# kabkabm/defensegan

Measured on NVIDIA H100. Metric: reconstructed images/sec at R=10,L=200, higher is better.
Workload: dtype f16

## Files before the change

### defensegan_b200/csrc/kernels_tc2.cuh

```cuda
#pragma once
#include "kernels_tc.cuh"
#include "tc_records.cuh"

namespace dgan {

constexpr int TC2_SMEM_MAX = 232448;
constexpr int TC2_TILE_BYTES = 128 * 128;
constexpr int TC2_BUF_COLS = 256;
constexpr int TC2_CONSUMERS = 256;
constexpr int TC2_THREADS = TC2_CONSUMERS + 128;
constexpr int TC2_PRODUCER_REGS = 40, TC2_CONSUMER_REGS = 232;
constexpr int TC2_STORE_ROWS = 16;

constexpr int TC2_MAX_PAIRS = 80;
struct Tc2Heads {
  uint32_t off[TC2_MAX_PAIRS + 1];
};

struct __align__(16) TcItem2 {
  uint16_t q[16];
  uint32_t n_acc;
};
static_assert(sizeof(TcItem2) == 48 && offsetof(TcItem2, n_acc) == 32, "the kernel's item loads");

__host__ __device__ constexpr int tc2_acc_stride(int n_tile) { return n_tile <= 32 ? 32 : (n_tile < 64 ? 64 : n_tile); }

__host__ __device__ constexpr bool tc2_tma_epilogue(int n_tile, int epi, int out_bytes) {
  return out_bytes == 2 && n_tile >= 64 && !tc_final_epi(epi);
}

constexpr int TC2_REC_BATCH = 16;
constexpr int TC2_STAGING_BYTES = TC2_REC_BATCH * (int)sizeof(TcRec);
constexpr int TC2_MREC_BYTES = TC2_NSLOT * (int)sizeof(TcRec);

__host__ __device__ constexpr int tc2_epi_tiles(int n_tile, int epi, int out_bytes) {
  return tc2_tma_epilogue(n_tile, epi, out_bytes) ? 2 : 0;
}
__host__ __device__ constexpr int tc2_ksub(int K) { return K % 64 == 0 ? 4 : K / 16; }
__host__ __device__ constexpr int tc2_a_bytes(int ksub) { return 128 * 32 * ksub; }
__host__ __device__ constexpr int tc2_b_bytes(int n_tile, int ksub) { return n_tile * 32 * ksub; }
__host__ __device__ constexpr bool tc2_issues_zero_ops(int maxb, int ksub) { return maxb > 4 || (maxb > 1 && ksub < 4); }
__host__ __device__ constexpr int tc2_zero_bytes(int n_tile, int maxb, int ksub) { return maxb > 1 ? tc2_b_bytes(n_tile, ksub) : 0; }
__host__ __device__ constexpr int tc2_ring_bytes(int n_tile, int maxb, int ksub, int epi, int out_bytes) {
  const int epi_b = tc2_epi_tiles(n_tile, epi, out_bytes) * TC2_TILE_BYTES;
  const int raw = ((TC2_SMEM_MAX - 1024 - 256 - TC2_MREC_BYTES - TC2_STAGING_BYTES - epi_b - tc2_zero_bytes(n_tile, maxb, ksub)) / 1024) * 1024;
  return raw > TC2_RING_MAX_KB * 1024 ? TC2_RING_MAX_KB * 1024 : raw;
}

template <int N_TILE, int MAXB_, int KSUB_ = 4, int EPI = EPI_NONE, int OUT_BYTES = 2>
struct Tc2Cfg {
  static_assert(MAXB_ >= 1 && MAXB_ <= TC2_BUF_COLS / tc2_acc_stride(N_TILE), "more accumulator slots than columns");
  static_assert(KSUB_ >= 1 && KSUB_ <= 4, "k16 MMAs per op");
  static constexpr int KSUB = KSUB_;
  static constexpr int A_BYTES = tc2_a_bytes(KSUB);
  static constexpr int B_TILE = tc2_b_bytes(N_TILE, KSUB);
  static constexpr int A_SUB = 128 * 32, B_SUB = N_TILE * 32;
  static constexpr int MAXB = MAXB_;
  static constexpr int ACC_REGS = MAXB * N_TILE / 2;
  static constexpr bool TMA_EPI = tc2_tma_epilogue(N_TILE, EPI, OUT_BYTES);
  static constexpr int EPI_TILES = tc2_epi_tiles(N_TILE, EPI, OUT_BYTES);
  static constexpr int EPI_BYTES = EPI_TILES * TC2_TILE_BYTES;
  static constexpr int ZERO_BYTES = tc2_zero_bytes(N_TILE, MAXB, KSUB);
  static constexpr int RING_BYTES = tc2_ring_bytes(N_TILE, MAXB, KSUB, EPI, OUT_BYTES);
  static constexpr int SMEM_BYTES = RING_BYTES + ZERO_BYTES + EPI_BYTES + TC2_STAGING_BYTES + 1024 + 256 + TC2_MREC_BYTES;
};

#define TC2_KINDS(X)                                                                                                   \
  X(256, 1, 4, EPI_BIAS_RELU, __half) X(256, 1, 4, EPI_BIAS, __half) X(256, 1, 4, EPI_MASK, __half)                    \
  X(256, 1, 4, EPI_NONE, __half) X(256, 1, 4, EPI_NONE, float) X(256, 1, 4, EPI_BIAS, float)                           \
  X(128, 2, 4, EPI_BIAS_RELU, __half) X(128, 2, 4, EPI_BIAS, __half) X(128, 2, 4, EPI_MASK, __half)                    \
  X(128, 2, 4, EPI_NONE, __half) X(128, 2, 4, EPI_NONE, float) X(128, 2, 4, EPI_BIAS, float)                           \
  X(128, 1, 4, EPI_NONE, float)                                                                                        \
  X(64, 4, 4, EPI_BIAS_RELU, __half) X(64, 4, 4, EPI_BIAS, __half) X(64, 4, 4, EPI_MASK, __half)                      \
  X(64, 4, 4, EPI_NONE, __half) X(64, 4, 4, EPI_NONE, float) X(64, 4, 4, EPI_BIAS, float)                              \
  X(64, 4, 1, EPI_MASK, __half) X(64, 4, 1, EPI_NONE, __half) X(64, 4, 3, EPI_NONE, __half)                            \
  X(128, 2, 1, EPI_MASK, __half) X(128, 2, 1, EPI_NONE, __half) X(128, 2, 3, EPI_NONE, __half)                         \
  X(16, 8, 4, EPI_FINAL_SIGMOID1, __half) X(16, 4, 4, EPI_FINAL_SIGMOID1, __half) X(48, 4, 4, EPI_FINAL_TANH3, __half)   \
  X(16, 8, 4, EPI_NONE, float) X(48, 4, 4, EPI_NONE, float)                                                              \
  X(16, 8, 4, EPI_FINAL_SIGMOID1_W, __half) X(16, 4, 4, EPI_FINAL_SIGMOID1_W, __half) X(48, 4, 4, EPI_FINAL_TANH3_W, __half)   \
  X(16, 8, 4, EPI_FINAL_SIGMOID1_H, __half) X(16, 4, 4, EPI_FINAL_SIGMOID1_H, __half) X(48, 4, 4, EPI_FINAL_TANH3_H, __half)   \
  X(16, 8, 4, EPI_FINAL_SIGMOID1_WH, __half) X(16, 4, 4, EPI_FINAL_SIGMOID1_WH, __half) X(48, 4, 4, EPI_FINAL_TANH3_WH, __half)

struct Tc2Kind { int n, maxb, ksub, epi, out_bytes; };
#define TC2_KIND_ROW(NT, MB, KS, EP, T) {NT, MB, KS, EP, (int)sizeof(T)},
static constexpr Tc2Kind kTc2Kinds[] = {TC2_KINDS(TC2_KIND_ROW)};
#undef TC2_KIND_ROW
constexpr bool tc2_kinds_fit_records() {
  for (const Tc2Kind& k : kTc2Kinds)
    if ((uint32_t)k.maxb > TcMmaRec::MaxB::mask || (uint32_t)k.ksub > TcMmaRec::Ksub::mask) return false;
  return true;
}
static_assert(tc2_kinds_fit_records(), "an instantiation's MAXB or KSUB does not fit the MMA record");
static inline bool tc2_has_kind(int n, int maxb, int ksub, int epi, int out_bytes) {
  for (const Tc2Kind& k : kTc2Kinds)
    if (k.n == n && k.maxb == maxb && k.ksub == ksub && k.epi == epi && k.out_bytes == out_bytes) return true;
  return false;
}

namespace ptx {
__device__ __forceinline__ void tma_store_3d(const CUtensorMap* map, uint32_t src, int c0, int c1, int c2) {
  asm volatile("cp.async.bulk.tensor.3d.global.shared::cta.tile.bulk_group [%0, {%2, %3, %4}], [%1];"
               ::"l"(map), "r"(src), "r"(c0), "r"(c1), "r"(c2) : "memory");
}
__device__ __forceinline__ void bulk_commit() { asm volatile("cp.async.bulk.commit_group;" ::: "memory"); }
__device__ __forceinline__ void bulk_wait_read1() { asm volatile("cp.async.bulk.wait_group.read 1;" ::: "memory"); }
__device__ __forceinline__ void bulk_wait_all0() { asm volatile("cp.async.bulk.wait_group 0;" ::: "memory"); }
__device__ __forceinline__ void fence_proxy_async_smem() { asm volatile("fence.proxy.async.shared::cta;" ::: "memory"); }
__device__ __forceinline__ uint32_t cluster_ctarank() {
  uint32_t r;
  asm volatile("mov.u32 %0, %%cluster_ctarank;" : "=r"(r));
  return r;
}
__device__ __forceinline__ void cluster_sync() {
  asm volatile("barrier.cluster.arrive.release.aligned;\n\tbarrier.cluster.wait.acquire.aligned;" ::: "memory");
}
__device__ __forceinline__ void tma_load_3d_mc2(uint32_t dst, const CUtensorMap* map, uint32_t bar, int c0, int c1, int c2) {
  asm volatile(
      "cp.async.bulk.tensor.3d.shared::cluster.global.mbarrier::complete_tx::bytes.multicast::cluster [%0], [%1, {%3, %4, %5}], [%2], %6;"
      ::"r"(dst), "l"(map), "r"(bar), "r"(c0), "r"(c1), "r"(c2), "h"((uint16_t)3) : "memory");
}
__device__ __forceinline__ void mbar_arrive_cluster(uint32_t local_bar, uint32_t cta) {
  asm volatile(
      "{\n\t.reg .b32 ra;\n\t"
      "mapa.shared::cluster.u32 ra, %0, %1;\n\t"
      "mbarrier.arrive.shared::cluster.b64 _, [ra];\n\t}" ::"r"(local_bar), "r"(cta) : "memory");
}
__device__ __forceinline__ void named_bar_sync(uint32_t id, uint32_t nthreads) {
  asm volatile("bar.sync %0, %1;" ::"r"(id), "r"(nthreads) : "memory");
}
__device__ __forceinline__ void st_shared_v4(uint32_t addr, uint32_t a, uint32_t b, uint32_t c, uint32_t d) {
  asm volatile("st.shared.v4.b32 [%0], {%1, %2, %3, %4};" ::"r"(addr), "r"(a), "r"(b), "r"(c), "r"(d) : "memory");
}
__device__ __forceinline__ void st_shared_u32(uint32_t addr, uint32_t v) { asm volatile("st.shared.b32 [%0], %1;" ::"r"(addr), "r"(v) : "memory"); }
__device__ __forceinline__ uint32_t ld_shared_u32(uint32_t addr) {
  uint32_t v;
  asm volatile("ld.shared.b32 %0, [%1];" : "=r"(v) : "r"(addr) : "memory");
  return v;
}
__device__ __forceinline__ uint2 ld_shared_v2(uint32_t addr) {
  uint2 v;
  asm volatile("ld.shared.v2.b32 {%0, %1}, [%2];" : "=r"(v.x), "=r"(v.y) : "r"(addr));
  return v;
}
__device__ __forceinline__ uint4 ld_shared_v4(uint32_t addr) {
  uint4 v;
  asm volatile("ld.shared.v4.b32 {%0, %1, %2, %3}, [%4];" : "=r"(v.x), "=r"(v.y), "=r"(v.z), "=r"(v.w) : "r"(addr));
  return v;
}
__device__ __forceinline__ uint4 ld_shared_v4_ordered(uint32_t addr) {
  uint4 v;
  asm volatile("ld.shared.v4.b32 {%0, %1, %2, %3}, [%4];" : "=r"(v.x), "=r"(v.y), "=r"(v.z), "=r"(v.w) : "r"(addr) : "memory");
  return v;
}
__device__ __forceinline__ void bulk_load(uint32_t dst, const void* src, uint32_t bytes, uint32_t bar) {
  asm volatile("cp.async.bulk.shared::cluster.global.mbarrier::complete_tx::bytes [%0], [%1], %2, [%3];"
               ::"r"(dst), "l"(src), "r"(bytes), "r"(bar) : "memory");
}
__device__ __forceinline__ void wgmma_wait1() { asm volatile("wgmma.wait_group.sync.aligned 1;" ::: "memory"); }
template <int R> __device__ __forceinline__ void setmaxnreg_inc() { asm volatile("setmaxnreg.inc.sync.aligned.u32 %0;" ::"n"(R)); }
template <int R> __device__ __forceinline__ void setmaxnreg_dec() { asm volatile("setmaxnreg.dec.sync.aligned.u32 %0;" ::"n"(R)); }
__device__ __forceinline__ bool elect_one() {
  uint32_t pred;
  asm volatile("{\n\t.reg .pred P1;\n\telect.sync _|P1, 0xffffffff;\n\tselp.u32 %0, 1, 0, P1;\n\t}" : "=r"(pred));
  return pred != 0;
}
}

__device__ __forceinline__ int tc2_item_at(const int* __restrict__ order, int k, int pair, int n_pairs, int n_slots) {
  return k < n_slots ? __ldg(order + (size_t)k * n_pairs + pair) : -1;
}

template <int NT, int MAXB, int KSUB, uint32_t MASK, int NREG>
__device__ __forceinline__ void tc2_mma_ops(float (&acc)[NREG], const uint32_t (&q)[6], uint64_t da0, uint64_t db0, uint32_t zoff) {
  constexpr uint32_t DA_K = KSUB == 4 ? 2u : (uint32_t)(128 * 32 >> 4), DB_K = KSUB == 4 ? 2u : (uint32_t)(NT * 32 >> 4);
#pragma unroll
  for (int a = 0; a < MAXB; ++a) {
    if (!((MASK >> a) & 1u)) continue;
    const uint32_t e = TcMmaRec::Ops::get(q[a / TcMmaRec::Ops::PER_WORD], a);
    const uint32_t bs = TcOp::Slot::get(e);
    const uint64_t da = da0 + (uint64_t)(TcOp::A::get(e) * (uint32_t)(tc2_a_bytes(KSUB) >> 4));
    const uint32_t boff = bs * (uint32_t)(tc2_b_bytes(NT, KSUB) >> 4);
    const uint64_t db = db0 + (uint64_t)(tc2_issues_zero_ops(MAXB, KSUB) && bs == (uint32_t)TC2_ZERO_SLOT ? zoff : boff);
    const uint32_t keep = TcOp::First::get(e) ^ 1u;
#pragma unroll
    for (int k = 0; k < KSUB; ++k) ptx::Wgmma<NT>::mma(acc + a * (NT / 2), da + DA_K * k, db + DB_K * k, k > 0 ? 1u : keep);
  }
  ptx::wgmma_commit();
}

template <int NT, int MAXB, int KSUB, int NREG>
__device__ __forceinline__ void tc2_mma_round(float (&acc)[NREG], const uint32_t (&q)[6], uint64_t da0, uint64_t db0, uint32_t zoff) {
  if constexpr (tc2_issues_zero_ops(MAXB, KSUB) || MAXB == 1) {
    tc2_mma_ops<NT, MAXB, KSUB, (1u << MAXB) - 1u>(acc, q, da0, db0, zoff);
  } else {
    static_assert(MAXB <= TcMmaRec::Ops::PER_WORD, "a round's op bytes share the queue's first word");
    uint32_t set = 0;
#pragma unroll
    for (int a = 0; a < MAXB; ++a)
      set |= (TcOp::Slot::get(TcMmaRec::Ops::get(q[0], a)) != (uint32_t)TC2_ZERO_SLOT ? 1u : 0u) << a;
    switch (set) {
#define TC2_ROUND_VARIANT(M) \
  case M:                    \
    if constexpr (M < (1u << MAXB)) tc2_mma_ops<NT, MAXB, KSUB, M>(acc, q, da0, db0, zoff); \
    break;
      TC2_ROUND_VARIANT(1u) TC2_ROUND_VARIANT(2u) TC2_ROUND_VARIANT(3u) TC2_ROUND_VARIANT(4u) TC2_ROUND_VARIANT(5u)
      TC2_ROUND_VARIANT(6u) TC2_ROUND_VARIANT(7u) TC2_ROUND_VARIANT(8u) TC2_ROUND_VARIANT(9u) TC2_ROUND_VARIANT(10u)
      TC2_ROUND_VARIANT(11u) TC2_ROUND_VARIANT(12u) TC2_ROUND_VARIANT(13u) TC2_ROUND_VARIANT(14u) TC2_ROUND_VARIANT(15u)
#undef TC2_ROUND_VARIANT
      default: __builtin_unreachable();
    }
  }
}

template <int MAXB>
__device__ __forceinline__ void tc2_pop_round(uint32_t (&q)[6]) {
  using Ops = TcMmaRec::Ops;
  static_assert(Ops::WORDS == 6, "the op queue holds every op word");
  if constexpr (MAXB >= Ops::PER_WORD) {
#pragma unroll
    for (int i = 0; i < 6; ++i) q[i] = (i + MAXB / Ops::PER_WORD < 6) ? q[i + MAXB / Ops::PER_WORD] : 0u;
  } else {
#pragma unroll
    for (int i = 0; i < 5; ++i) q[i] = __funnelshift_r(q[i], q[i + 1], Ops::BITS * MAXB);
    q[5] >>= Ops::BITS * MAXB;
  }
}

#ifdef DGAN_PROBE
constexpr int TC2_PROBE_WORDS = 18;
__device__ unsigned long long g_tc2_probe[48][160][TC2_PROBE_WORDS];
__device__ __forceinline__ unsigned long long probe_gtime() {
  unsigned long long t;
  asm volatile("mov.u64 %0, %%globaltimer;" : "=l"(t));
  return t;
}
__device__ __forceinline__ long long probe_clock_after(uint32_t w0) {
  long long t;
  asm volatile("{\n\t.reg .pred p;\n\tsetp.ge.s32 p, %1, 0;\n\tmov.u64 %0, 0;\n\t@p mov.u64 %0, %%clock64;\n\t}" : "=l"(t) : "r"(w0) : "memory");
  return t;
}
__device__ __forceinline__ long long probe_clock_after64(unsigned long long v) {
  long long t;
  asm volatile("{\n\t.reg .pred p;\n\tsetp.eq.u64 p, %1, 0;\n\t@p mov.u64 %0, %%clock64;\n\t@!p mov.u64 %0, %%clock64;\n\t}"
               : "=l"(t) : "l"(v) : "memory");
  return t;
}
__device__ __forceinline__ unsigned long long probe_bits(float2 v) {
  return ((unsigned long long)__float_as_uint(v.y) << 32) | __float_as_uint(v.x);
}
__host__ __device__ constexpr int tc2_probe_key(int n_tile, int epi, int out_bytes) {
  if (epi >= EPI_FINAL_SIGMOID1_H) return 40 + epi - EPI_FINAL_SIGMOID1_H;
  return (n_tile == 256 ? 0 : n_tile == 128 ? 1 : n_tile == 64 ? 2 : n_tile == 48 ? 3 : 4) * 8 + (out_bytes == 4 ? 6 : (epi < 4 ? epi : epi - 4));
}
#endif

template <int N_TILE, int MAXB, int KSUB, int EPI, typename TOUT>
__global__ void __cluster_dims__(2, 1, 1) __launch_bounds__(TC2_THREADS, 1)
tc_bsgemm2_kernel(const __grid_constant__ CUtensorMap tm_a, const __grid_constant__ CUtensorMap tm_b,
                  const __grid_constant__ CUtensorMap tm_out,
                  const TcItem2* __restrict__ items, const TcRec* __restrict__ stream_p,
                  const TcRec* __restrict__ stream_m, const __grid_constant__ Tc2Heads heads,
                  const int* __restrict__ eitems, int n_slots,
                  TOUT* __restrict__ out, int n_pad, const float* __restrict__ bias, int bias_pstride, const TcFinalArgs fa) {
  using Cfg = Tc2Cfg<N_TILE, MAXB, KSUB, EPI, (int)sizeof(TOUT)>;
  constexpr bool TMA_EPI = Cfg::TMA_EPI;
  constexpr bool HUBER = (EPI == EPI_FINAL_SIGMOID1_H || EPI == EPI_FINAL_TANH3_H || EPI == EPI_FINAL_SIGMOID1_WH ||
                          EPI == EPI_FINAL_TANH3_WH);
  constexpr bool WEIGHTED = (EPI == EPI_FINAL_SIGMOID1_W || EPI == EPI_FINAL_TANH3_W || EPI == EPI_FINAL_SIGMOID1_WH ||
                             EPI == EPI_FINAL_TANH3_WH);
  constexpr bool FINAL = tc_final_epi(EPI);
  constexpr bool SIGMOID1 = (EPI == EPI_FINAL_SIGMOID1 || EPI == EPI_FINAL_SIGMOID1_W || EPI == EPI_FINAL_SIGMOID1_H ||
                             EPI == EPI_FINAL_SIGMOID1_WH);
  constexpr bool HAS_BIAS = (EPI == EPI_BIAS_RELU || EPI == EPI_BIAS);
  constexpr int B_TILE = Cfg::B_TILE, A_BYTES = Cfg::A_BYTES;
  constexpr int PRODUCER = TC2_CONSUMERS / 32;
  extern __shared__ uint8_t smem_raw[];
#ifdef DGAN_PROBE
  const long long probe_t_start = clock64();
  const unsigned long long probe_g_start = probe_gtime();
  long long probe_wait_full = 0, probe_issue = 0, probe_wait1 = 0, probe_wait0 = 0, probe_epi = 0, probe_in = 0, probe_stage = 0;
  unsigned probe_rec = 0, probe_head = 0, probe_steps = 0;
#endif
  const uint32_t smem_base = (ptx::smem_u32(smem_raw) + 1023u) & ~1023u;
  const uint32_t zero_base = smem_base + Cfg::RING_BYTES;
  const uint32_t epi_base = zero_base + Cfg::ZERO_BYTES;
  const uint32_t stg_base = epi_base + Cfg::EPI_BYTES;
  const uint32_t bar_base = stg_base + TC2_STAGING_BYTES;
  const uint32_t bar_full = bar_base, bar_empty = bar_base + 64, mrec_base = bar_base + 256;

  const int warp = threadIdx.x >> 5, lane = threadIdx.x & 31;
  const uint32_t rank = ptx::cluster_ctarank();
  const int pair = blockIdx.x >> 1, n_pairs = gridDim.x >> 1;
  const uint32_t rbeg = heads.off[pair], rend = heads.off[pair + 1];

  uint4 mine = make_uint4(0, 0, 0, 0);
  if (warp == PRODUCER) {
    if (2 * rbeg + lane < 2 * rend) mine = __ldg(reinterpret_cast<const uint4*>(stream_p + rbeg) + lane);
    if (lane == 0) {
      ptx::prefetch_tmap(&tm_a);
      ptx::prefetch_tmap(&tm_b);
      if (TMA_EPI) ptx::prefetch_tmap(&tm_out);
      for (int s = 0; s < TC2_NSLOT; ++s) {
        ptx::mbar_init(bar_full + 8 * s, 1);
        ptx::mbar_init(bar_empty + 8 * s, 2 * TC2_CONSUMERS / 32);
      }
      ptx::fence_barrier_init();
    }
  }
  if constexpr (Cfg::ZERO_BYTES > 0 && tc2_issues_zero_ops(MAXB, KSUB)) {
    if (threadIdx.x < TC2_CONSUMERS) {
      for (uint32_t i = threadIdx.x; i < (uint32_t)Cfg::ZERO_BYTES / 16u; i += TC2_CONSUMERS) ptx::st_shared_v4(zero_base + 16u * i, 0u, 0u, 0u, 0u);
      ptx::fence_proxy_async_smem();
    }
  }
  ptx::cluster_sync();
#ifdef DGAN_PROBE
  const long long probe_t_entry = clock64();
#endif
  pdl_launch_dependents();
  pdl_wait();
#ifdef DGAN_PROBE
  const long long probe_t_go = clock64();
  unsigned probe_h0 = (unsigned)probe_t_go;
  bool probe_new_item = true;
#endif

  if (warp >= PRODUCER) {
    ptx::setmaxnreg_dec<TC2_PRODUCER_REGS>();
    if (warp == PRODUCER) {
      const TcRec* __restrict__ stream = stream_p;
      uint32_t it = 0;
      const uint32_t ring = stg_base;
      for (uint32_t base = rbeg; base < rend; base += TC2_REC_BATCH) {
        ptx::st_shared_v4(ring + lane * 16u, mine.x, mine.y, mine.z, mine.w);
        __syncwarp();
        if (2 * (base + TC2_REC_BATCH) + lane < 2 * rend) mine = __ldg(reinterpret_cast<const uint4*>(stream + base + TC2_REC_BATCH) + lane);
        const uint32_t cnt = min((uint32_t)TC2_REC_BATCH, rend - base);
        for (uint32_t i = 0; i < cnt; ++i, ++it) {
          const uint4 r0 = ptx::ld_shared_v4(ring + i * 32u);
          const uint2 r1 = ptx::ld_shared_v2(ring + i * 32u + 16u);
          const uint32_t slot = it & (TC2_NSLOT - 1);
          using P = TcProducerRec;
          const int kc = P::Kc::get(r0.x), nA = P::NA::get(r0.x), nB = P::NB::get(r0.x);
          const uint32_t dep = (r0.x >> P::Dep::shift) & P::Dep::mask;
          const int row0 = (2 * (int)P::Mp::get(r0.y) + (int)rank) * kRowTile;
          if (it >= dep) ptx::mbar_wait(bar_empty + 8 * ((it - dep) & (TC2_NSLOT - 1)), ((it - dep) >> 3) & 1);
          if (dep != TC2_NSLOT && it >= TC2_NSLOT) ptx::mbar_wait(bar_empty + 8 * slot, ((it - TC2_NSLOT) >> 3) & 1);
          const uint32_t full = bar_full + 8 * slot;
          const uint32_t sa = smem_base + (P::Off::get(r0.x) << 10);
          if (ptx::elect_one()) {
            ptx::mbar_expect_tx(full, (uint32_t)(nA * A_BYTES + nB * B_TILE) + (uint32_t)sizeof(TcRec));
            ptx::bulk_load(mrec_base + slot * (uint32_t)sizeof(TcRec), stream_m + rbeg + it, (uint32_t)sizeof(TcRec), full);
#pragma unroll
            for (int a = 0; a < TC2_MAX_A; ++a) {
              if (a >= nA) break;
              const int p = (int)P::Pix::get(a < P::Pix::PER_WORD ? r0.z : r0.w, a);
              if constexpr (KSUB == 4) {
                ptx::tma_load_3d(sa + a * A_BYTES, &tm_a, full, kc * 64, row0, p);
              } else {
#pragma unroll
                for (int k = 0; k < KSUB; ++k)
                  ptx::tma_load_3d(sa + a * A_BYTES + k * Cfg::A_SUB, &tm_a, full, (kc * KSUB + k) * 16, row0, p);
              }
            }
            const uint32_t sb = sa + nA * A_BYTES;
#pragma unroll
            for (int b = 0; b < TC2_MAX_BSLOTS; ++b) {
              if (b >= nB) break;
              const uint32_t t = P::Tile::get(b < P::Tile::PER_WORD ? r1.x : r1.y, b);
              if constexpr (KSUB == 4) {
                ptx::tma_load_3d_mc2(sb + b * B_TILE + rank * (B_TILE / 2), &tm_b, full, kc * 64, (int)rank * (N_TILE / 2), (int)t);
              } else {
#pragma unroll
                for (int k = 0; k < KSUB; ++k)
                  ptx::tma_load_3d_mc2(sb + b * B_TILE + k * Cfg::B_SUB + rank * (Cfg::B_SUB / 2), &tm_b, full, (kc * KSUB + k) * 16,
                                       (int)rank * (N_TILE / 2), (int)t);
              }
            }
          }
          __syncwarp();
        }
        __syncwarp();
      }
      for (uint32_t j = it > TC2_NSLOT ? it - TC2_NSLOT : 0; j < it; ++j) ptx::mbar_wait(bar_empty + 8 * (j & (TC2_NSLOT - 1)), (j >> 3) & 1);
    }
  } else {
    ptx::setmaxnreg_inc<TC2_CONSUMER_REGS>();
    const int wg = warp >> 2, wl = warp & 3;
    const int r_lo = wg * 64 + wl * 16 + (lane >> 2);
    float acc[Cfg::ACC_REGS];
#pragma unroll
    for (int i = 0; i < Cfg::ACC_REGS; ++i) acc[i] = 0.f;
    uint32_t item_count = 0, store_count = 0;
    uint32_t ri = rbeg, it = 0;
    auto item_desc = [&](int e, int& n, uint32_t& qm) {
      n = 0; qm = 0u;
      if (e < 0) return;
      const TcItem2* ip = items + tc2_item_window(e);
      n = (int)__ldg(&ip->n_acc);
      if (lane < 16) qm = (uint32_t)__ldg(&ip->q[lane]);
    };
    int e_cur = tc2_item_at(eitems, 0, pair, n_pairs, n_slots), e_nx = tc2_item_at(eitems, 1, pair, n_pairs, n_slots), n_acc_cur;
    uint32_t q_cur;
    item_desc(e_cur, n_acc_cur, q_cur);
    constexpr bool BIAS_CH = HAS_BIAS && TMA_EPI && N_TILE < 256, BIAS_PX = HAS_BIAS && TMA_EPI && !BIAS_CH;
    static_assert(!BIAS_CH || (Cfg::ZERO_BYTES >= N_TILE * 4 && !tc2_issues_zero_ops(MAXB, KSUB)), "the bias copy's space");
    static_assert(!BIAS_PX || MAXB == 1, "a per-pixel bias is held for one accumulator");
    if constexpr (BIAS_CH) {
      if (threadIdx.x < N_TILE / 2) {
        const float2 b2 = __ldg(reinterpret_cast<const float2*>(bias) + threadIdx.x);
        ptx::st_shared_u32(zero_base + 8u * threadIdx.x, __float_as_uint(b2.x));
        ptx::st_shared_u32(zero_base + 8u * threadIdx.x + 4u, __float_as_uint(b2.y));
      }
      ptx::named_bar_sync(4, TC2_CONSUMERS);
    }
    constexpr int CO = SIGMOID1 ? 1 : 3, FJ = FINAL ? N_TILE / 8 : 1;
    constexpr bool FINAL_PREFETCH = !(WEIGHTED && N_TILE > 32);
    constexpr int FINAL_HELD = FINAL && N_TILE <= 32 && !(WEIGHTED && MAXB > 4) ? MAXB : 1;
    const int hwc = fa.w_out * fa.w_out * CO;
    float bsv[CO];
    if constexpr (FINAL) {
#pragma unroll
      for (int co = 0; co < CO; ++co) bsv[co] = __ldg(bias + co);
    }
    while (ri < rend) {
      const int item_e = e_cur, n_acc = n_acc_cur;
      const uint32_t q_mine = q_cur;
      const int mp = tc2_item_mp(item_e);
      const int tile_row0 = (2 * mp + (int)rank) * kRowTile;
      const size_t n_lo = (size_t)(tile_row0 + r_lo);
      constexpr int G_UNITS = TMA_EPI ? N_TILE / 64 : 1;
      static_assert(EPI != EPI_MASK || MAXB * G_UNITS == 4, "one mask unit per lane of a quad");
      unsigned long long mk_pre[2] = {~0ull, ~0ull};
// ... 26 lines not shown
          xv[j] = make_float2(0.f, 0.f);
          if (fa.x != nullptr) xv[j] = __ldg(reinterpret_cast<const float2*>(fa.x + (size_t)img * hwc + off));
          wv[j] = make_float2(1.f, 1.f);
          if (WEIGHTED) wv[j] = __ldg(reinterpret_cast<const float2*>(fa.xw + (size_t)img * hwc + off));
        }
      };
      float2 xp[FINAL_HELD][2][FJ], wp[FINAL_HELD][2][FJ];
      if constexpr (FINAL && FINAL_PREFETCH) {
#pragma unroll
        for (int a = 0; a < FINAL_HELD; ++a) {
          if (a >= n_acc) break;
          final_pairs(a, 0, xp[a][0], wp[a][0]);
          final_pairs(a, 1, xp[a][1], wp[a][1]);
        }
      }
      item_desc(e_nx, n_acc_cur, q_cur);
      e_cur = e_nx;
      e_nx = tc2_item_at(eitems, (int)item_count + 2, pair, n_pairs, n_slots);
      uint32_t flags;
      do {
        const uint32_t slot = it & (TC2_NSLOT - 1), phase = (it >> 3) & 1;
#ifdef DGAN_PROBE
        const long long probe_w0 = clock64();
        if (probe_new_item) probe_head += (unsigned)probe_w0 - probe_h0;
        probe_new_item = false;
#endif
        ptx::mbar_wait(bar_full + 8 * slot, phase);
#ifdef DGAN_PROBE
        const long long probe_w1 = clock64();
        probe_wait_full += probe_w1 - probe_w0;
        if (it == 0 && threadIdx.x == 0) g_tc2_probe[tc2_probe_key(N_TILE, EPI, (int)sizeof(TOUT))][blockIdx.x][7] = probe_gtime();
#endif
        const uint4 r0 = ptx::ld_shared_v4_ordered(mrec_base + slot * (uint32_t)sizeof(TcRec));
        const uint4 r1 = ptx::ld_shared_v4_ordered(mrec_base + slot * (uint32_t)sizeof(TcRec) + 16u);
        flags = TcMmaRec::Flags::get(r0.x);
#ifdef DGAN_PROBE
        const unsigned probe_rec_step = (unsigned)probe_clock_after(r0.x) - (unsigned)probe_w1;
        probe_rec += probe_rec_step;
#endif
        const int nA = TcMmaRec::NA::get(r0.x), n_rounds = TcMmaRec::Rounds::get(r0.x);
        const uint32_t sa = smem_base + (TcMmaRec::Off::get(r0.x) << 10);
        const uint64_t da0 = KSUB == 4 ? make_smem_desc_sw128(sa + (uint32_t)wg * 64u * 128u) : make_smem_desc_sw32(sa + (uint32_t)wg * 64u * 32u);
        const uint32_t sb = sa + (uint32_t)nA * A_BYTES;
        const uint64_t db0 = KSUB == 4 ? make_smem_desc_sw128(sb) : make_smem_desc_sw32(sb);
        const uint32_t zoff = (zero_base - sb) >> 4;
        uint32_t q[6] = {r0.z, r0.w, r1.x, r1.y, r1.z, r1.w};
#ifdef DGAN_PROBE
        long long probe_step_wait = 0;
#endif
        ptx::fence_operands(acc);
        ptx::wgmma_fence();
        for (int r = 0; r < n_rounds; ++r) {
          tc2_mma_round<N_TILE, Cfg::MAXB, KSUB>(acc, q, da0, db0, zoff);
          tc2_pop_round<Cfg::MAXB>(q);
#ifdef DGAN_PROBE
          const long long probe_c0 = clock64();
#endif
          ptx::wgmma_wait1();
#ifdef DGAN_PROBE
          probe_step_wait += clock64() - probe_c0;
#endif
          if (r == 0) {
            __syncwarp();
            if (!(flags & TcMmaRec::FIRST) && lane < 2) ptx::mbar_arrive_cluster(bar_empty + 8 * ((it - 1) & (TC2_NSLOT - 1)), (uint32_t)lane);
          }
        }
        ptx::fence_operands(acc);
#ifdef DGAN_PROBE
        probe_wait1 += probe_step_wait;
        probe_issue += clock64() - probe_w1 - probe_step_wait - probe_rec_step;
#endif
        ++ri; ++it;
      } while (!(flags & TcMmaRec::LAST));
#ifdef DGAN_PROBE
      const long long probe_d0 = clock64();
#endif
      ptx::wgmma_wait0();
      ptx::fence_operands(acc);
#ifdef DGAN_PROBE
      const long long probe_e0 = clock64();
      probe_wait0 += probe_e0 - probe_d0;
#endif
      __syncwarp();
      if (lane < 2) ptx::mbar_arrive_cluster(bar_empty + 8 * ((it - 1) & (TC2_NSLOT - 1)), (uint32_t)lane);

      auto q_of = [&](int a) { return (int)__shfl_sync(0xffffffffu, q_mine, a); };
      if constexpr (FINAL) {
#pragma unroll
        for (int a = 0; a < Cfg::MAXB; ++a) {
          if (a >= n_acc) break;
          const int blk = q_of(a);
          const int by = blk / fa.nbx, bx = blk % fa.nbx;
#ifdef DGAN_PROBE
          const long long probe_a0 = clock64();
#endif
#pragma unroll
          for (int h = 0; h < 2; ++h) {
            float2 xa[FJ], wa[FJ];
            if constexpr (FINAL_PREFETCH) {
#pragma unroll
              for (int j = 0; j < FJ; ++j) { xa[j] = xp[a % FINAL_HELD][h][j]; wa[j] = wp[a % FINAL_HELD][h][j]; }
              if (FINAL_HELD == 1 && a + 1 < Cfg::MAXB && a + 1 < n_acc) final_pairs(a + 1, h, xp[0][h], wp[0][h]);
            } else {
              final_pairs(a, h, xa, wa);
            }
#ifdef DGAN_PROBE
            if (h == 0) probe_in += probe_clock_after64(probe_bits(xa[0]) ^ probe_bits(wa[0])) - probe_a0;
#endif
            const size_t n = n_lo + 8 * h;
            float lsum = 0.f;
#pragma unroll
            for (int j = 0; j < N_TILE / 8; ++j) {
              const int col = j * 8 + (lane & 3) * 2;
              const int li = col / (4 * CO), e = col % (4 * CO);
              const size_t off = (size_t)((4 * by + li) * fa.w_out + 4 * bx) * CO + e;
              const float2 xv = xa[j], wv = wa[j];
              float yv[2], dv[2];
#pragma unroll
              for (int c = 0; c < 2; ++c) {
                const float pre = acc[a * (N_TILE / 2) + j * 4 + h * 2 + c] + bsv[(e + c) % CO];
                float yy, dact;
                if (SIGMOID1) { yy = __fdividef(1.f, 1.f + __expf(-pre)); dact = yy * (1.f - yy); }
                else { const float t = __expf(-2.f * fabsf(pre)); yy = copysignf(__fdividef(1.f - t, 1.f + t), pre); dact = 1.f - yy * yy; }
                yv[c] = yy;
                float d = 0.f;
                if (HUBER) {
                  d = yy - (c ? xv.y : xv.x);
                  const float cl = fabsf(d) > fa.huber ? copysignf(fa.huber, d) : d;
                  const float ew = WEIGHTED ? (c ? wv.y : wv.x) * cl : cl;
                  lsum = fmaf(ew, 2.f * d - cl, lsum);
                  d = ew;
                } else if (WEIGHTED) {
                  d = yy - (c ? xv.y : xv.x);
                  const float ew = (c ? wv.y : wv.x) * d;
                  lsum = fmaf(ew, d, lsum);
                  d = ew;
                } else if (fa.x != nullptr) { d = yy - (c ? xv.y : xv.x); lsum = fmaf(d, d, lsum); }
                dv[c] = d * dact * fa.gscale;
              }
              if (fa.write_y) *reinterpret_cast<float2*>(fa.y + n * hwc + off) = make_float2(yv[0], yv[1]);
              if (fa.x != nullptr)
                *reinterpret_cast<uint32_t*>(reinterpret_cast<__half*>(out) + ((size_t)blk * n_pad + n) * N_TILE + col) = pack_half2(dv[0], dv[1]);
            }
            lsum += __shfl_xor_sync(0xffffffffu, lsum, 1);
            lsum += __shfl_xor_sync(0xffffffffu, lsum, 2);
            if (fa.x != nullptr && fa.write_y && (lane & 3) == 0) fa.loss_part[(size_t)blk * n_pad + n] = lsum;
          }
        }
      } else if constexpr (TMA_EPI) {
        constexpr int G = N_TILE / 64;
        const int GT = fa.out_ld >> 6;
        const int row_w = tile_row0 + wg * 64 + wl * 16;
        const uint32_t s_warp = epi_base + (uint32_t)warp * 4096u;
        const uint32_t swz = (uint32_t)(lane >> 2);
#pragma unroll
        for (int a = 0; a < Cfg::MAXB; ++a) {
          if (a >= n_acc) break;
          const int q = q_of(a);
#pragma unroll
          for (int g = 0; g < G; ++g) {
#ifdef DGAN_PROBE
            const long long probe_u0 = clock64();
#endif
            unsigned long long mk[2] = {~0ull, ~0ull}, bits[2] = {0ull, 0ull};
            if (EPI == EPI_MASK) {
#pragma unroll
              for (int h = 0; h < 2; ++h) mk[h] = __shfl_sync(0xffffffffu, mk_pre[h], (lane & ~3) | (a * G + g));
#ifdef DGAN_PROBE
              probe_in += probe_clock_after64(mk[0] ^ mk[1]) - probe_u0;
#endif
            }
            uint32_t pk[2][8];
#pragma unroll
            for (int j = 0; j < 8; ++j) {
              const int cl = j * 8 + (lane & 3) * 2;
              float2 bv = make_float2(0.f, 0.f);
              if constexpr (BIAS_CH) {
                const uint2 b2 = ptx::ld_shared_v2(zero_base + (uint32_t)(g * 64 + cl) * 4u);
                bv = make_float2(__uint_as_float(b2.x), __uint_as_float(b2.y));
              }
              if constexpr (BIAS_PX) {
                bv.x = __shfl_sync(0xffffffffu, bias_px[g].x, j * 4 + (lane & 3));
                bv.y = __shfl_sync(0xffffffffu, bias_px[g].y, j * 4 + (lane & 3));
              }
#ifdef DGAN_PROBE
              if (HAS_BIAS && j == 0) probe_in += probe_clock_after64(probe_bits(bv)) - probe_u0;
#endif
#pragma unroll
              for (int h = 0; h < 2; ++h) {
                float v0 = acc[a * (N_TILE / 2) + (g * 8 + j) * 4 + h * 2];
                float v1 = acc[a * (N_TILE / 2) + (g * 8 + j) * 4 + h * 2 + 1];
                if (HAS_BIAS) { v0 += bv.x; v1 += bv.y; }
                if (EPI == EPI_BIAS_RELU) {
                  v0 = fmaxf(v0, 0.f); v1 = fmaxf(v1, 0.f);
                  bits[h] |= ((unsigned long long)(v0 > 0.f) << cl) | ((unsigned long long)(v1 > 0.f) << (cl + 1));
                }
                if (EPI == EPI_MASK) {
                  if (!((mk[h] >> cl) & 1ull)) v0 = 0.f;
                  if (!((mk[h] >> (cl + 1)) & 1ull)) v1 = 0.f;
                }
                pk[h][j] = pack_half2(v0, v1);
              }
            }
            const uint32_t buf = s_warp + (store_count & 1u) * 2048u;
#ifdef DGAN_PROBE
            const long long probe_s0 = clock64();
#endif
            if (lane == 0) ptx::bulk_wait_read1();
            __syncwarp();
#ifdef DGAN_PROBE
            probe_stage += clock64() - probe_s0;
#endif
#pragma unroll
            for (int h = 0; h < 2; ++h)
#pragma unroll
              for (int j = 0; j < 8; ++j)
                ptx::st_shared_u32(buf + (swz + 8u * h) * 128u + (((uint32_t)j ^ swz) << 4) + (uint32_t)(lane & 3) * 4u, pk[h][j]);
            ptx::fence_proxy_async_smem();
            __syncwarp();
            if (lane == 0) {
              ptx::tma_store_3d(&tm_out, buf, fa.col0 + g * 64, row_w, q);
              ptx::bulk_commit();
            }
            ++store_count;
            if (EPI == EPI_BIAS_RELU && fa.mb_out != nullptr) {
#pragma unroll
              for (int h = 0; h < 2; ++h) {
                bits[h] |= __shfl_xor_sync(0xffffffffu, bits[h], 1);
                bits[h] |= __shfl_xor_sync(0xffffffffu, bits[h], 2);
              }
              if ((lane & 3) < 2) fa.mb_out[((size_t)q * n_pad + n_lo + 8 * (lane & 1)) * GT + g] = (lane & 1) ? bits[1] : bits[0];
            }
          }
        }
      } else {
#pragma unroll
        for (int a = 0; a < Cfg::MAXB; ++a) {
          if (a >= n_acc) break;
          const int q = q_of(a);
#pragma unroll
          for (int j = 0; j < N_TILE / 8; ++j) {
            const int col = j * 8 + (lane & 3) * 2;
            float2 bv = make_float2(0.f, 0.f);
            if (HAS_BIAS) bv = __ldg(reinterpret_cast<const float2*>(bias + (size_t)q * bias_pstride + col));
#pragma unroll
            for (int h = 0; h < 2; ++h) {
              float v0 = acc[a * (N_TILE / 2) + j * 4 + h * 2] + bv.x, v1 = acc[a * (N_TILE / 2) + j * 4 + h * 2 + 1] + bv.y;
              if (EPI == EPI_BIAS_RELU) { v0 = fmaxf(v0, 0.f); v1 = fmaxf(v1, 0.f); }
              const size_t o = ((size_t)q * n_pad + n_lo + 8 * h) * fa.out_ld + col;
              if (sizeof(TOUT) == 4) *reinterpret_cast<float2*>(reinterpret_cast<float*>(out) + o) = make_float2(v0, v1);
              else *reinterpret_cast<uint32_t*>(reinterpret_cast<__half*>(out) + o) = pack_half2(v0, v1);
            }
          }
        }
      }
      if (EPI == EPI_NONE && sizeof(TOUT) == 4 && fa.m_counter != nullptr) {
        const uint32_t flag_addr = bar_base + 200;
        const unsigned rt = 2u * (unsigned)mp + rank;
        __threadfence();
        ptx::named_bar_sync(3, TC2_CONSUMERS);
        if (threadIdx.x == 0) {
          const unsigned ticket = atomicAdd(fa.m_counter + rt, 1u);
          ptx::st_shared_u32(flag_addr, ticket == (unsigned)TC_LINEAR_SPLIT - 1u ? 1u : 0u);
        }
        ptx::named_bar_sync(3, TC2_CONSUMERS);
        if (ptx::ld_shared_u32(flag_addr) != 0u) {
          __threadfence();
          const float* __restrict__ gp = reinterpret_cast<const float*>(out);
          const size_t base = (size_t)rt * kRowTile * N_TILE;
          const int tid = threadIdx.x;
          constexpr int STRIDE = 4 * TC2_CONSUMERS, UNR = 4;
          for (int e0 = tid * 4; e0 < kRowTile * N_TILE; e0 += UNR * STRIDE) {
            float4 gs[UNR], vv[UNR], zz[UNR];
#pragma unroll
            for (int u = 0; u < UNR; ++u) {
              const size_t i = base + (size_t)(e0 + u * STRIDE);
              gs[u] = __ldcg(reinterpret_cast<const float4*>(gp + i));
              vv[u] = *reinterpret_cast<const float4*>(fa.mv + i);
              zz[u] = *reinterpret_cast<const float4*>(fa.mz + i);
            }
            float4 t[TC_LINEAR_SPLIT - 1][UNR];
#pragma unroll
            for (int pp = 1; pp < TC_LINEAR_SPLIT; ++pp)
#pragma unroll
              for (int u = 0; u < UNR; ++u)
                t[pp - 1][u] = __ldcg(reinterpret_cast<const float4*>(gp + base + (size_t)(e0 + u * STRIDE) + (size_t)pp * fa.m_count));
#pragma unroll
            for (int pp = 1; pp < TC_LINEAR_SPLIT; ++pp)
#pragma unroll
              for (int u = 0; u < UNR; ++u) { gs[u].x += t[pp - 1][u].x; gs[u].y += t[pp - 1][u].y; gs[u].z += t[pp - 1][u].z; gs[u].w += t[pp - 1][u].w; }
#pragma unroll
            for (int u = 0; u < UNR; ++u) {
              const size_t i = base + (size_t)(e0 + u * STRIDE);
              float4 v4 = vv[u], z4 = zz[u];
              v4.x = fmaf(fa.m_mu, v4.x, fa.m_gmul * gs[u].x); v4.y = fmaf(fa.m_mu, v4.y, fa.m_gmul * gs[u].y);
              v4.z = fmaf(fa.m_mu, v4.z, fa.m_gmul * gs[u].z); v4.w = fmaf(fa.m_mu, v4.w, fa.m_gmul * gs[u].w);
              z4.x -= fa.m_lr * v4.x; z4.y -= fa.m_lr * v4.y; z4.z -= fa.m_lr * v4.z; z4.w -= fa.m_lr * v4.w;
              *reinterpret_cast<float4*>(fa.mv + i) = v4;
              *reinterpret_cast<float4*>(fa.mz + i) = z4;
              if (fa.mz_h != nullptr)
                *reinterpret_cast<uint2*>(fa.mz_h + i) = make_uint2(pack_half2(z4.x, z4.y), pack_half2(z4.z, z4.w));
            }
          }
          if (tid == 0) fa.m_counter[rt] = 0u;
        }
      }
#ifdef DGAN_PROBE
      const long long probe_e1 = clock64();
      probe_epi += probe_e1 - probe_e0;
      probe_h0 = (unsigned)probe_e1;
      probe_new_item = true;
      probe_steps = it;
#endif
      ++item_count;
    }
    if (TMA_EPI && lane == 0) ptx::bulk_wait_all0();
  }

#ifdef DGAN_PROBE
  {
    constexpr int key = tc2_probe_key(N_TILE, EPI, (int)sizeof(TOUT));
    if (threadIdx.x == 0) {
      atomicAdd(&g_tc2_probe[key][blockIdx.x][3], (unsigned long long)probe_wait_full);
      atomicAdd(&g_tc2_probe[key][blockIdx.x][8], (unsigned long long)probe_issue);
      atomicAdd(&g_tc2_probe[key][blockIdx.x][9], (unsigned long long)probe_wait1);
      atomicAdd(&g_tc2_probe[key][blockIdx.x][10], (unsigned long long)probe_wait0);
      atomicAdd(&g_tc2_probe[key][blockIdx.x][11], (unsigned long long)probe_epi);
      atomicAdd(&g_tc2_probe[key][blockIdx.x][16], (unsigned long long)probe_in);
      atomicAdd(&g_tc2_probe[key][blockIdx.x][17], (unsigned long long)probe_stage);
    }
    __syncthreads();
    if (threadIdx.x == 0) {
      atomicAdd(&g_tc2_probe[key][blockIdx.x][12], (unsigned long long)probe_rec);
      atomicAdd(&g_tc2_probe[key][blockIdx.x][13], (unsigned long long)probe_head);
      atomicAdd(&g_tc2_probe[key][blockIdx.x][15], (unsigned long long)probe_steps);
      if (probe_steps != 0) atomicAdd(&g_tc2_probe[key][blockIdx.x][14], (unsigned long long)((unsigned)clock64() - probe_h0));
      atomicAdd(&g_tc2_probe[key][blockIdx.x][0], (unsigned long long)(clock64() - probe_t_go));
      atomicAdd(&g_tc2_probe[key][blockIdx.x][1], 1ull);
      atomicAdd(&g_tc2_probe[key][blockIdx.x][2], (unsigned long long)(probe_t_go - probe_t_entry));
      atomicAdd(&g_tc2_probe[key][blockIdx.x][4], (unsigned long long)(probe_t_entry - probe_t_start));
      g_tc2_probe[key][blockIdx.x][5] = probe_g_start;
      g_tc2_probe[key][blockIdx.x][6] = probe_gtime();
    }
  }
#endif
  ptx::cluster_sync();
}

struct Tc2Schedule {
  TcItem2* items = nullptr;
  TcRec* stream_p = nullptr;
  TcRec* stream_m = nullptr;
  Tc2Heads heads{};
  int* eitems = nullptr;
  int n_slots = 0, n_pairs = 0;
  int maxb = 1;
};
static uint32_t tc2_box_k(int K) { return tc2_ksub(K) == 4 ? 64u : 16u; }
struct TcDir {
  std::string name, kind;
  int N = 0, K = 0, P_in = 0, P_out = 0, n_tiles = 0;
  PairTable tab;
  int h_grid = 0, w_grid = 0;
  int max_acc = 1;
  int epi = EPI_NONE, out_bytes = 2, bias_pstride = 0;
  int ld = 0, col0 = 0, out_ld = 0;
  int n_real = 0;
  std::string base_kind;
  __half* w = nullptr;
  CUtensorMap tm_b{};
  int force_maxb = 0;
  std::vector<std::pair<int, Tc2Schedule>> by_mpairs;
};

static int tc2_maxb(int N) { return TC2_BUF_COLS / tc2_acc_stride(N); }

struct Tc2HostStep {
  int kc = 0, nA = 0, nB = 0, n_rounds = 0;
  int a_pix[TC2_MAX_A] = {0, 0, 0, 0};
  uint8_t b_ent[TC2_MAX_BSLOTS] = {0};
  uint8_t ops[TC2_OP_BYTES] = {0};
  int n_real = 0;
  int bytes = 0;
};
struct Tc2HostItem {
  TcItem2 hdr{};
  std::vector<Tc2HostStep> steps;
  double stage_bytes = 0.0;
  long long n_ops = 0;
  long long n_issued = 0;
};

static void tc2_build_item(const PairTable& tab, const std::vector<int>& qs, int N, int K, int max_b, int max_a,
                           int step_max_bytes, Tc2HostItem* out) {
  const int ksub = tc2_ksub(K), kch = K / (16 * ksub), a_bytes = tc2_a_bytes(ksub), b_tile = tc2_b_bytes(N, ksub);
  out->hdr = TcItem2{};
  out->hdr.n_acc = (uint32_t)qs.size();
  for (size_t a = 0; a < qs.size(); ++a) out->hdr.q[a] = (uint16_t)qs[a];
  out->steps.clear();
  std::vector<std::pair<int, std::vector<std::pair<int, int>>>> by_p;
  for (size_t a = 0; a < qs.size(); ++a)
    for (int e = tab.off[qs[a]]; e < tab.off[qs[a] + 1]; ++e) {
      const int p = tab.pairs[e].x, t = tab.pairs[e].y;
      size_t g = 0;
      for (; g < by_p.size(); ++g)
        if (by_p[g].first == p) break;
      if (g == by_p.size()) by_p.push_back({p, {}});
      by_p[g].second.push_back({t, (int)a});
    }
  std::sort(by_p.begin(), by_p.end(), [](const auto& l, const auto& r) { return l.first < r.first; });
  for (auto& g : by_p)
    std::stable_sort(g.second.begin(), g.second.end(), [](const auto& l, const auto& r) { return l.second < r.second; });
  std::vector<std::pair<int, std::vector<std::pair<int, int>>>> px;
  const int ent_cap = std::min(TC2_MAX_BSLOTS, std::max(1, (step_max_bytes - a_bytes) / b_tile));
  for (auto& g : by_p)
    for (size_t b0 = 0; b0 < g.second.size(); b0 += (size_t)ent_cap)
      px.push_back({g.first, std::vector<std::pair<int, int>>(g.second.begin() + b0,
                                                               g.second.begin() + std::min(g.second.size(), b0 + (size_t)ent_cap))});
  const int max_rounds = TC2_OP_BYTES / max_b;
  struct Group { size_t i0, i1; };
  std::vector<Group> groups;
  {
    size_t i0 = 0;
    while (i0 < px.size()) {
      size_t i1 = i0;
      std::vector<int> staged;
      int cnt[8] = {0, 0, 0, 0, 0, 0, 0, 0};
      auto have = [&](int t) { return std::find(staged.begin(), staged.end(), t) != staged.end(); };
      while (i1 < px.size() && (int)(i1 - i0) < max_a) {
        int fresh = 0;
        std::vector<int> fresh_tiles;
        int c2[8];
        std::copy(cnt, cnt + 8, c2);
        int rounds = 0;
        for (auto& ta : px[i1].second) {
          if (!have(ta.first) && std::find(fresh_tiles.begin(), fresh_tiles.end(), ta.first) == fresh_tiles.end()) {
            fresh_tiles.push_back(ta.first); ++fresh;
          }
          ++c2[ta.second];
        }
        for (int a = 0; a < 8; ++a) rounds = std::max(rounds, c2[a]);
        const int nA = (int)(i1 - i0) + 1, nB = (int)staged.size() + fresh;
        const bool dup_pixel = (i1 > i0 && px[i1].first == px[i1 - 1].first);
        if (i1 > i0 && (dup_pixel || nB > TC2_MAX_BSLOTS || rounds > max_rounds ||
                        nA * a_bytes + nB * b_tile > step_max_bytes))
          break;
        for (int t : fresh_tiles) staged.push_back(t);
        std::copy(c2, c2 + 8, cnt);
        ++i1;
      }
      groups.push_back({i0, i1});
      i0 = i1;
    }
  }
  uint32_t seen = 0;
  for (size_t gi = 0; gi < groups.size(); ++gi) {
    const Group& G = groups[gi];
    Tc2HostStep st;
    st.nA = (int)(G.i1 - G.i0);
    std::fill(st.ops, st.ops + TC2_OP_BYTES, TC2_PAD_OP);
    int slot_of[32], cnt[8] = {0, 0, 0, 0, 0, 0, 0, 0};
    for (int t = 0; t < 32; ++t) slot_of[t] = -1;
    for (size_t i = G.i0; i < G.i1; ++i) {
      st.a_pix[i - G.i0] = px[i].first;
      for (auto& ta : px[i].second) {
        const int t = ta.first, acc = ta.second;
        if (slot_of[t] < 0) {
          slot_of[t] = st.nB;
          st.b_ent[st.nB++] = (uint8_t)t;
        }
        const bool first = !(seen & (1u << acc));
        const int r = cnt[acc]++;
        st.ops[r * max_b + acc] = TcOp{(uint32_t)(i - G.i0), (uint32_t)slot_of[t], first ? 1u : 0u}.encode();
        st.n_rounds = std::max(st.n_rounds, r + 1);
        st.n_real += 1;
        seen |= 1u << acc;
      }
    }
    st.bytes = st.nA * a_bytes + st.nB * b_tile;
    out->steps.push_back(st);
  }
  const size_t n_groups = out->steps.size();
// ... 436 lines not shown
```

Measured before the change: 2798.

## Stage TMA epilogue tiles with stmatrix and compute masks with byte permutes

The TMA-store epilogue now writes its swizzled staging tile with four stmatrix.x4 instructions instead of sixteen scalar shared stores per lane. Masking is done with prmt-built halfword masks applied to the packed half2 values. ReLU sign bits are gathered into 32-bit words with two shuffles and written in one batch after all tiles, rather than as 64-bit shuffled stores inside the loop. This is meant to cut shared-store instruction count and the per-tile shuffle and global-store work, at the cost of extra registers for the buffered mask words. It also adds probe counters.

```diff
diff --git a/defensegan_b200/csrc/kernels_tc2.cuh b/defensegan_b200/csrc/kernels_tc2.cuh
--- a/defensegan_b200/csrc/kernels_tc2.cuh
+++ b/defensegan_b200/csrc/kernels_tc2.cuh
@@ -106,6 +106,14 @@
 __device__ __forceinline__ void bulk_wait_read1() { asm volatile("cp.async.bulk.wait_group.read 1;" ::: "memory"); }
 __device__ __forceinline__ void bulk_wait_all0() { asm volatile("cp.async.bulk.wait_group 0;" ::: "memory"); }
 __device__ __forceinline__ void fence_proxy_async_smem() { asm volatile("fence.proxy.async.shared::cta;" ::: "memory"); }
+__device__ __forceinline__ void stmatrix_x4(uint32_t addr, uint32_t a, uint32_t b, uint32_t c, uint32_t d) {
+  asm volatile("stmatrix.sync.aligned.m8n8.x4.shared.b16 [%0], {%1, %2, %3, %4};" ::"r"(addr), "r"(a), "r"(b), "r"(c), "r"(d) : "memory");
+}
+__device__ __forceinline__ uint32_t prmt(uint32_t a, uint32_t b, uint32_t sel) {
+  uint32_t r;
+  asm("prmt.b32 %0, %1, %2, %3;" : "=r"(r) : "r"(a), "r"(b), "r"(sel));
+  return r;
+}
 __device__ __forceinline__ uint32_t cluster_ctarank() {
   uint32_t r;
   asm volatile("mov.u32 %0, %%cluster_ctarank;" : "=r"(r));
@@ -227,7 +235,7 @@
 }
 
 #ifdef DGAN_PROBE
-constexpr int TC2_PROBE_WORDS = 18;
+constexpr int TC2_PROBE_WORDS = 21;
 __device__ unsigned long long g_tc2_probe[48][160][TC2_PROBE_WORDS];
 __device__ __forceinline__ unsigned long long probe_gtime() {
   unsigned long long t;
@@ -279,6 +287,7 @@
   const long long probe_t_start = clock64();
   const unsigned long long probe_g_start = probe_gtime();
   long long probe_wait_full = 0, probe_issue = 0, probe_wait1 = 0, probe_wait0 = 0, probe_epi = 0, probe_in = 0, probe_stage = 0;
+  long long probe_regs = 0, probe_sts = 0, probe_fence = 0;
   unsigned probe_rec = 0, probe_head = 0, probe_steps = 0;
 #endif
   const uint32_t smem_base = (ptx::smem_u32(smem_raw) + 1023u) & ~1023u;
@@ -611,7 +620,10 @@
         const int GT = fa.out_ld >> 6;
         const int row_w = tile_row0 + wg * 64 + wl * 16;
         const uint32_t s_warp = epi_base + (uint32_t)warp * 4096u;
-        const uint32_t swz = (uint32_t)(lane >> 2);
+        const uint32_t l2 = 2u * (uint32_t)(lane & 3);
+        const uint32_t sm_row = (uint32_t)(lane & 7) + 8u * (uint32_t)((lane >> 3) & 1);
+        const uint32_t sm_x = (((uint32_t)(lane >> 4) ^ (uint32_t)(lane & 7)) << 4);
+        uint32_t mw[Cfg::MAXB * G];
 #pragma unroll
         for (int a = 0; a < Cfg::MAXB; ++a) {
           if (a >= n_acc) break;
@@ -619,17 +631,27 @@
 #pragma unroll
           for (int g = 0; g < G; ++g) {
 #ifdef DGAN_PROBE
-            const long long probe_u0 = clock64();
-#endif
-            unsigned long long mk[2] = {~0ull, ~0ull}, bits[2] = {0ull, 0ull};
-            if (EPI == EPI_MASK) {
+            const long long probe_u0 = clock64(), probe_in0 = probe_in;
+#endif
+            uint32_t keep7[2][2], keep6[2][2];
+            if constexpr (EPI == EPI_MASK) {
+              unsigned long long mk[2];
 #pragma unroll
               for (int h = 0; h < 2; ++h) mk[h] = __shfl_sync(0xffffffffu, mk_pre[h], (lane & ~3) | (a * G + g));
 #ifdef DGAN_PROBE
               probe_in += probe_clock_after64(mk[0] ^ mk[1]) - probe_u0;
 #endif
+#pragma unroll
+              for (int h = 0; h < 2; ++h)
+#pragma unroll
+                for (int hi = 0; hi < 2; ++hi) {
+                  const uint32_t w = (uint32_t)(mk[h] >> (32 * hi));
+                  keep7[h][hi] = w << (7u - l2);
+                  keep6[h][hi] = w << (6u - l2);
+                }
             }
             uint32_t pk[2][8];
+            uint32_t bits[2][2] = {{0u, 0u}, {0u, 0u}};
 #pragma unroll
             for (int j = 0; j < 8; ++j) {
               const int cl = j * 8 + (lane & 3) * 2;
@@ -651,46 +673,70 @@
                 float v1 = acc[a * (N_TILE / 2) + (g * 8 + j) * 4 + h * 2 + 1];
                 if (HAS_BIAS) { v0 += bv.x; v1 += bv.y; }
                 if (EPI == EPI_BIAS_RELU) {
+                  const uint32_t b = 8u * (uint32_t)(j & 3);
+                  if (v0 > 0.f) bits[h][j >> 2] |= 1u << b;
+                  if (v1 > 0.f) bits[h][j >> 2] |= 2u << b;
                   v0 = fmaxf(v0, 0.f); v1 = fmaxf(v1, 0.f);
-                  bits[h] |= ((unsigned long long)(v0 > 0.f) << cl) | ((unsigned long long)(v1 > 0.f) << (cl + 1));
-                }
-                if (EPI == EPI_MASK) {
-                  if (!((mk[h] >> cl) & 1ull)) v0 = 0.f;
-                  if (!((mk[h] >> (cl + 1)) & 1ull)) v1 = 0.f;
                 }
                 pk[h][j] = pack_half2(v0, v1);
+                if (EPI == EPI_MASK) pk[h][j] &= ptx::prmt(keep7[h][j >> 2], keep6[h][j >> 2], 0xCC88u + 0x1111u * (uint32_t)(j & 3));
               }
             }
+            if constexpr (EPI == EPI_BIAS_RELU) {
+              const bool up = (lane & 2) != 0, odd = (lane & 1) != 0;
+              uint32_t k0 = (up ? bits[1][0] : bits[0][0]) << l2, k1 = (up ? bits[1][1] : bits[0][1]) << l2;
+              const uint32_t s0 = (up ? bits[0][0] : bits[1][0]) << l2, s1 = (up ? bits[0][1] : bits[1][1]) << l2;
+              k0 |= __shfl_xor_sync(0xffffffffu, s0, 2);
+              k1 |= __shfl_xor_sync(0xffffffffu, s1, 2);
+              mw[a * G + g] = (odd ? k1 : k0) | __shfl_xor_sync(0xffffffffu, odd ? k0 : k1, 1);
+            }
             const uint32_t buf = s_warp + (store_count & 1u) * 2048u;
 #ifdef DGAN_PROBE
-            const long long probe_s0 = clock64();
+            const long long probe_s0 = probe_clock_after64((((unsigned long long)pk[0][7] << 32) | pk[1][7]) ^
+                                                           (EPI == EPI_BIAS_RELU ? mw[a * G + g] : 0u));
+            probe_regs += probe_s0 - probe_u0 - (probe_in - probe_in0);
 #endif
             if (lane == 0) ptx::bulk_wait_read1();
             __syncwarp();
 #ifdef DGAN_PROBE
-            probe_stage += clock64() - probe_s0;
-#endif
-#pragma unroll
-            for (int h = 0; h < 2; ++h)
-#pragma unroll
-              for (int j = 0; j < 8; ++j)
-                ptx::st_shared_u32(buf + (swz + 8u * h) * 128u + (((uint32_t)j ^ swz) << 4) + (uint32_t)(lane & 3) * 4u, pk[h][j]);
+            const long long probe_s1 = clock64();
+            probe_stage += probe_s1 - probe_s0;
+#endif
+#pragma unroll
+            for (int p = 0; p < 4; ++p)
+              ptx::stmatrix_x4(buf + sm_row * 128u + ((32u * (uint32_t)p) ^ sm_x), pk[0][2 * p], pk[1][2 * p], pk[0][2 * p + 1], pk[1][2 * p + 1]);
+#ifdef DGAN_PROBE
+            const long long probe_f0 = clock64();
+            probe_sts += probe_f0 - probe_s1;
+#endif
             ptx::fence_proxy_async_smem();
+#ifdef DGAN_PROBE
+            probe_fence += clock64() - probe_f0;
+#endif
             __syncwarp();
             if (lane == 0) {
               ptx::tma_store_3d(&tm_out, buf, fa.col0 + g * 64, row_w, q);
               ptx::bulk_commit();
             }
             ++store_count;
-            if (EPI == EPI_BIAS_RELU && fa.mb_out != nullptr) {
-#pragma unroll
-              for (int h = 0; h < 2; ++h) {
-                bits[h] |= __shfl_xor_sync(0xffffffffu, bits[h], 1);
-                bits[h] |= __shfl_xor_sync(0xffffffffu, bits[h], 2);
-              }
-              if ((lane & 3) < 2) fa.mb_out[((size_t)q * n_pad + n_lo + 8 * (lane & 1)) * GT + g] = (lane & 1) ? bits[1] : bits[0];
-            }
           }
+        }
+        if (EPI == EPI_BIAS_RELU && fa.mb_out != nullptr) {
+#ifdef DGAN_PROBE
+          const long long probe_m0 = clock64();
+#endif
+          uint32_t* __restrict__ mb32 = reinterpret_cast<uint32_t*>(fa.mb_out);
+          const size_t row = n_lo + 8 * ((lane >> 1) & 1);
+#pragma unroll
+          for (int a = 0; a < Cfg::MAXB; ++a) {
+            if (a >= n_acc) break;
+            const int q = q_of(a);
+#pragma unroll
+            for (int g = 0; g < G; ++g) mb32[(((size_t)q * n_pad + row) * GT + g) * 2 + (lane & 1)] = mw[a * G + g];
+          }
+#ifdef DGAN_PROBE
+          probe_regs += clock64() - probe_m0;
+#endif
         }
       } else {
 #pragma unroll
@@ -787,6 +833,9 @@
       atomicAdd(&g_tc2_probe[key][blockIdx.x][11], (unsigned long long)probe_epi);
       atomicAdd(&g_tc2_probe[key][blockIdx.x][16], (unsigned long long)probe_in);
       atomicAdd(&g_tc2_probe[key][blockIdx.x][17], (unsigned long long)probe_stage);
+      atomicAdd(&g_tc2_probe[key][blockIdx.x][18], (unsigned long long)probe_regs);
+      atomicAdd(&g_tc2_probe[key][blockIdx.x][19], (unsigned long long)probe_sts);
+      atomicAdd(&g_tc2_probe[key][blockIdx.x][20], (unsigned long long)probe_fence);
     }
     __syncthreads();
     if (threadIdx.x == 0) {
```

After: 2890 (median of 6 runs). +3.3%, better.
